# shubhamchandak94/HARC

Hardware: AMD Instinct MI355X
Metric: Mreads/s reorder+encode, 100 bp (higher is better)
Workload: dtype u64 (2-bit packed bases, XOR+popcount)

## Files before the change

harc_amd/csrc/stage2.hip:

```cpp
#include "devutil.h"
#include <time.h>
#include <algorithm>
#include <stdlib.h>

#define TUPLE_NONE 0xFFFFFFFFFFFFFFFFULL

struct S2Args {
    int L, W, W3, thresh_s, maxsearch;
    int ds[2], de[2], kbits[2];
    uint32_t M, S, T, q, nC;
    uint64_t total;
    const uint64_t *oreads;
    const uint8_t *flag, *pos, *rc;
    const uint32_t *order;
    const uint64_t *cand3;
    const uint32_t *cand_order;
    uint8_t *head;
    uint64_t *gstart;
    uint8_t *cons;
    const uint32_t *chead;
    const HashSlot *slots[2]; uint64_t cap[2]; const uint32_t *ids[2];
    unsigned long long *best;
    unsigned long long *bestbin[2];
    const uint32_t *bloom[2]; int bloom_shift[2];
    int bloom_lbits, bloom_nwin;
    const uint64_t *cons2;
    const uint64_t *cand2, *candN;
    uint4 *events;
    unsigned int *nevents; uint32_t maxevents;
    int trace;
    uint64_t col0, col1; uint32_t tile_base;
    const uint64_t *evwin;
    unsigned long long *cbb[2]; uint32_t *cpos[2], *ccnt[2]; unsigned long long *tminbin[2]; int compact;
    int binmax_on;
    unsigned long long *binmax[2];
};

__device__ __forceinline__ int base2_at(const uint64_t *r, int j) { return (int)((r[j >> 5] >> (2 * (j & 31))) & 3); }
__device__ __forceinline__ int pc_to_idx(int pc) { return ((pc & 1) << 1) | (pc >> 1); }
__device__ __forceinline__ int c3_at(const uint64_t *r, int W3, int j)
{
    const int off = 3 * j, wi = off >> 6, sh = off & 63;
    uint64_t v = r[wi] >> sh;
    if (sh > 61 && wi + 1 < W3) v |= r[wi + 1] << (64 - sh);
    return (int)(v & 7);
}
__device__ __forceinline__ int c3_to_idx5(int c3) { return c3 == 0 ? 0 : c3 == 4 ? 1 : c3 == 2 ? 2 : c3 == 6 ? 3 : 4; }
__device__ __forceinline__ int idx_to_c3(int idx) { return idx == 0 ? 0 : idx == 1 ? 4 : idx == 2 ? 2 : 6; }
__device__ __forceinline__ int comp5(int b) { return b == 4 ? 4 : 3 - b; }
__device__ __forceinline__ char enc_noise(int ref, int rd)
{
    const unsigned tabA = 0x32100, tabC = 0x32100, tabG = 0x30021, tabT = 0x30012;
    const unsigned t = ref == 0 ? tabA : ref == 1 ? tabC : ref == 2 ? tabG : tabT;
    return (char)('0' + ((t >> (4 * rd)) & 0xF));
}
__device__ __forceinline__ long long ub_le(const uint64_t *a, long long n, uint64_t x)
{
    long long lo = -1, hi = n;
    while (hi - lo > 1) { const long long mid = (lo + hi) >> 1; if (a[mid] <= x) lo = mid; else hi = mid; }
    return lo;
}

__global__ void k_cand3_from2(const uint64_t *reads2, const uint32_t *gather, uint32_t n, int L, int W, int W3, uint64_t *out)
{
    const size_t gid = harc_gid();
    if (gid >= (size_t)n * W3) return;
    const uint32_t i = (uint32_t)(gid / W3); const int w = (int)(gid % W3);
    const uint64_t *r = reads2 + (size_t)(gather ? gather[i] : i) * W;
    uint64_t v = 0;
    const int b0 = (64 * w) / 3, b1 = (64 * w + 63) / 3;
    for (int b = b0; b <= b1 && b < L; b++) {
        const uint64_t c3 = (uint64_t)(2 * base2_at(r, b));
        const int sh = 3 * b - 64 * w;
        v |= sh >= 0 ? (c3 << sh) : (c3 >> (-sh));
    }
    out[gid] = v;
}
__global__ void k_cand_order(const uint32_t *order_s, uint32_t S, uint32_t T, uint32_t *out)
{
    const uint32_t i = harc_gid32();
    if (i >= T) return;
    out[i] = i < S ? order_s[i] : i - S;
}
__global__ void k_key3(const uint64_t *cand3, uint32_t T, int W3, int off, int nbits, uint64_t *keys, uint32_t *ids)
{
    const uint32_t i = harc_gid32();
    if (i >= T) return;
    const uint64_t *r = cand3 + (size_t)i * W3;
    const int wi = off >> 6, sh = off & 63;
    uint64_t v = r[wi] >> sh;
    if (sh && wi + 1 < W3) v |= r[wi + 1] << (64 - sh);
    if (nbits < 64) v &= ((uint64_t)1 << nbits) - 1;
    keys[i] = v; ids[i] = i;
}
__global__ void k_count_big_bins(const HashSlot *slots, uint64_t cap, uint32_t maxsearch, unsigned long long *out)
{
    const uint64_t i = harc_gid();
    if (i >= cap) return;
    if ((slots[i].count & SLOT_CNT_MASK) > maxsearch) atomicAdd(out, 1ULL);
}

__global__ void k_heads1(const uint8_t *flag, uint32_t M, uint32_t q, uint8_t *head, uint32_t *hidx)
{
    const uint32_t i = harc_gid32();
    if (i >= M) return;
    const uint8_t h = (flag[i] == '0' || (i % q) == 0) ? 1 : 0;
    head[i] = h; hidx[i] = h ? i : 0;
}
__global__ void k_heads2(uint32_t M, uint8_t *head, const uint32_t *hmax, uint32_t *hidx)
{
    const uint32_t i = harc_gid32();
    if (i >= M) return;
// ... 249 lines not shown
    lh ^= lh >> 15; lh *= 0x85EBCA77u; lh ^= lh >> 13;
    *word = ((lh >> (32 - lbits)) << 4) | ((kh >> 6) & 15u);
    *sh0 = 4 * (int)(kh & 7u); *sh1 = 4 * (int)((kh >> 3) & 7u);
}
__global__ void k_bloom4_set(const uint64_t *keys, uint32_t n, uint32_t *bloom, int lbits, int nwin, int l, int nb)
{
    const uint32_t i = harc_gid32();
    if (i >= n) return;
    const uint64_t k = keys[i];
    uint64_t f = 0, r = 0;
    for (int b = 0; b < nb; b++) {
        const uint32_t c3 = (uint32_t)(k >> (3 * b)) & 7u;
        if (c3 & 1u) return;
        const uint64_t idx = ((c3 >> 2) & 1u) | (c3 & 2u);
        f |= idx << (2 * b); r |= (3u - idx) << (2 * (nb - 1 - b));
    }
    uint32_t w; int a, b;
    bloom4_pos(f, bloom4_minimizer(f, nwin), nwin, lbits, &w, &a, &b);
    atomicOr(&bloom[w], ((1u << l) << a) | ((1u << l) << b));
    bloom4_pos(r, bloom4_minimizer(r, nwin), nwin, lbits, &w, &a, &b);
    atomicOr(&bloom[w], ((4u << l) << a) | ((4u << l) << b));
}
__global__ void k_bloom4_items(const uint64_t *keys, uint32_t n, int lbits, int nwin, int l, int nb, uint32_t skip_tile, uint64_t *items)
{
    const uint32_t i = harc_gid32();
    if (i >= n) return;
    const uint64_t k = keys[i];
    uint64_t f = 0, r = 0; bool hasn = false;
    for (int b = 0; b < nb; b++) {
        const uint32_t c3 = (uint32_t)(k >> (3 * b)) & 7u;
        hasn |= (c3 & 1u) != 0;
        const uint64_t idx = ((c3 >> 2) & 1u) | (c3 & 2u);
        f |= idx << (2 * b); r |= (3u - idx) << (2 * (nb - 1 - b));
    }
    if (hasn) { items[2 * (size_t)i] = items[2 * (size_t)i + 1] = (uint64_t)skip_tile; return; }
    uint32_t w; int a, b;
    bloom4_pos(f, bloom4_minimizer(f, nwin), nwin, lbits, &w, &a, &b);
    items[2 * (size_t)i] = harc_bitmap_item(w, a + l, b + l);
    bloom4_pos(r, bloom4_minimizer(r, nwin), nwin, lbits, &w, &a, &b);
    items[2 * (size_t)i + 1] = harc_bitmap_item(w, a + 2 + l, b + 2 + l);
}
__global__ void k_words_differ(const uint32_t *a, const uint32_t *b, uint64_t nwords, unsigned long long *ndiff)
{
    const uint64_t i = harc_gid();
    const unsigned long long m = __ballot(i < nwords && a[i] != b[i]);
    if ((threadIdx.x & 63) == 0 && m) atomicAdd(ndiff, (unsigned long long)__popcll(m));
}
__global__ void k_cand2_from3(const uint64_t *cand3, uint32_t T, int L, int W, int W3, uint64_t *cand2, uint64_t *candN)
{
    const uint64_t gid = harc_gid();
    if (gid >= (uint64_t)T * W) return;
    const uint32_t i = (uint32_t)(gid / W); const int w = (int)(gid % W);
    const uint64_t *r = cand3 + (size_t)i * W3;
    (void)L;
    const int wi = (3 * w) >> 1;
    const uint64_t x0 = r[wi], x1 = wi + 1 < W3 ? r[wi + 1] : 0;
    uint64_t lo, hi;
    if (w & 1) { lo = (x0 >> 32) | (x1 << 32); hi = x1 >> 32; } else { lo = x0; hi = x1 & 0xFFFFFFFFull; }
    uint64_t a = 0, n = 0;
#pragma unroll
    for (int k = 0; k < 32; k++) {
        const uint64_t c3 = (k <= 20 ? (lo >> (3 * k)) : k == 21 ? ((lo >> 63) | (hi << 1)) : (hi >> (3 * k - 64))) & 7;
        a |= (c3 >> 1) << (2 * k);
        n |= ((c3 & 1) * 3) << (2 * k);
    }
    cand2[gid] = a; candN[gid] = n;
}
template <int W> __device__ __forceinline__ void cons_words(const uint64_t *cons2, uint64_t g, uint64_t (&cw)[W])
{
    const uint64_t bit = 2 * g, wi = bit >> 6; const int sh = (int)(bit & 63);
    uint64_t lo = cons2[wi];
#pragma unroll
    for (int w = 0; w < W; w++) { const uint64_t hi = cons2[wi + w + 1]; cw[w] = sh ? ((lo >> sh) | (hi << (64 - sh))) : lo; lo = hi; }
}

#define RSTRIP 8
#define RTILE (256 * RSTRIP)
static_assert(RTILE == CTILE, "the proposal kernels are launched on the consensus kernel's tiles");
template <int W> __device__ __forceinline__ void realign_probe(const S2Args &s, uint64_t x, int dir, int l, uint64_t key)
{
    uint32_t st = 0, cnt = 0;
    if (!dict_lookup_b(s.slots[l], s.cap[l], key, &st, &cnt)) return;
    const int L = s.L;
    const unsigned long long tp = (x << 2) | ((uint64_t)dir << 1) | (uint64_t)l;
    if (cnt & SLOT_BIG) {
        const unsigned int at = atomicAdd(s.nevents, 1u);
        if (at < s.maxevents) s.events[at] = make_uint4((uint32_t)tp, (uint32_t)(tp >> 32), st, cnt & SLOT_CNT_MASK);
        return;
    }
    uint64_t wv[W];
    {
        uint64_t cw[W];
        cons_words<W>(s.cons2, x, cw);
#pragma unroll
        for (int w = 0; w < W; w++) cw[w] &= lowmask_word(2 * L, w);
        if (dir) rc_words<W>(cw, L, wv);
        else {
#pragma unroll
            for (int w = 0; w < W; w++) wv[w] = cw[w];
        }
    }
    const bool emb = (cnt & SLOT_EMB) != 0;
    cnt &= SLOT_CNT_MASK;
    for (uint32_t t = 0; t < cnt; t++) {
        const uint32_t rid = emb ? st : s.ids[l][st + cnt - 1 - t];
        const uint64_t *a2 = s.cand2 + (size_t)rid * W, *n2 = s.candN + (size_t)rid * W;
        int hd = 0;
#pragma unroll
        for (int w = 0; w < W; w++) {
            const uint64_t av = a2[w], nv = n2[w];
            hd += __popcll((av ^ wv[w]) & ~nv) + __popcll(nv & 0x5555555555555555ULL) + __popcll(wv[w] & nv);
        }
        if (hd <= s.thresh_s) atomicMin(&s.best[rid], tp);
    }
}
#define RQCAP 4096
template <int W> __device__ __forceinline__ void realign_hit1(const S2Args &s, const uint8_t *tile, uint64_t X0, int tc, int p, int n)
{
    const int dir = p >> 1, l = p & 1;
    const uint64_t cpos = X0 + tc;
    const uint64_t off = dir ? (uint64_t)(s.L - 1 - s.de[l]) : (uint64_t)s.ds[l];
    if (cpos < off) return;
    const uint64_t x = cpos - off;
    if (x < s.col0 || x >= s.col1 || !(s.cons[x] & 4)) return;
    uint64_t key = 0;
    if (dir) for (int b = 0; b < n; b++) key |= (uint64_t)idx_to_c3(3 - (tile[tc + n - 1 - b] & 3)) << (3 * b);
    else for (int b = 0; b < n; b++) key |= (uint64_t)idx_to_c3(tile[tc + b] & 3) << (3 * b);
    realign_probe<W>(s, x, dir, l, key);
}
template <int W, int NWIN> __global__ __launch_bounds__(256) void k_realign_propose1(S2Args s)
{
    __shared__ uint32_t tile32[(RTILE + 64 + 8) / 4];
    __shared__ uint16_t queue[RQCAP];
    __shared__ uint2 lookup[RTILE];
    __shared__ unsigned int qn;
    uint8_t *tile = reinterpret_cast<uint8_t *>(tile32);
    const uint64_t X0 = (uint64_t)(blockIdx.x + s.tile_base) * RTILE;
    const int n = s.de[0] - s.ds[0] + 1;
    const int ntile = RTILE + n + NWIN + 1;
    for (int d = threadIdx.x; d < (ntile + 3) / 4; d += 256) {
        const uint64_t g = X0 + 4ull * d;
        uint32_t v = 0;
        if (g + 4 <= s.total) v = *reinterpret_cast<const uint32_t *>(s.cons + g);
        else for (int k = 0; k < 4; k++) if (g + k < s.total) v |= (uint32_t)s.cons[g + k] << (8 * k);
        tile32[d] = v;
    }
    if (threadIdx.x == 0) qn = 0;
    __syncthreads();
    const int t0 = threadIdx.x * RSTRIP;
    uint64_t k = 0;
    for (int b = 0; b < n; b++) k |= (uint64_t)(tile[t0 + b] & 3) << (2 * b);
    const uint32_t *bloom = s.bloom[0]; const int lbits = s.bloom_lbits;
    constexpr int NK = RSTRIP + (NWIN > 0 ? NWIN - 1 : 0);
    uint64_t keys[RSTRIP]; uint32_t mm[NK];
#pragma unroll
    for (int c = 0; c < NK; c++) {
        if (c < RSTRIP) keys[c] = k;
        mm[c] = bloom4_mmer(k);
        k = (k >> 2) | ((uint64_t)(tile[t0 + c + n] & 3) << (2 * (n - 1)));
    }
#pragma unroll
    for (int c = 0; c < RSTRIP; c++) {
        uint32_t mz = 0xFFFFFFFFu;
#pragma unroll
        for (int i = 0; i < NWIN; i++) mz = mm[c + i] < mz ? mm[c + i] : mz;
        uint32_t w; int a, b;
        bloom4_pos(keys[c], mz, NWIN, lbits, &w, &a, &b);
        lookup[t0 + c] = make_uint2(w, (uint32_t)a | ((uint32_t)b << 8));
    }
    __syncthreads();
#pragma unroll
    for (int c = 0; c < RSTRIP; c++) {
        const int col = c * 256 + (int)threadIdx.x;
        if (X0 + col < s.total) {
            const uint2 lk = lookup[col];
            const uint32_t v = bloom[lk.x];
            uint32_t m = (v >> (lk.y & 0xFFu)) & (v >> (lk.y >> 8)) & 15u;
            while (m) {
                const int p = __builtin_ctz(m); m &= m - 1;
                const unsigned int at = atomicAdd(&qn, 1u);
                if (at < RQCAP) queue[at] = (uint16_t)(col | (p << 12));
                else realign_hit1<W>(s, tile, X0, col, p, n);
            }
        }
    }
    __syncthreads();
    const unsigned int nq = qn < RQCAP ? qn : RQCAP;
    for (unsigned int i = threadIdx.x; i < nq; i += 256) { const uint16_t e = queue[i]; realign_hit1<W>(s, tile, X0, e & 0xFFF, e >> 12, n); }
}

template <int W> __global__ __launch_bounds__(256) void k_realign_propose(S2Args s)
{
    __shared__ uint32_t tile32[(RTILE + 256 + 8) / 4];
    uint8_t *tile = reinterpret_cast<uint8_t *>(tile32);
    const uint64_t X0 = (uint64_t)(blockIdx.x + s.tile_base) * RTILE;
    const int L = s.L;
    const int ntile = RTILE + L + 1;
    for (int d = threadIdx.x; d < (ntile + 3) / 4; d += 256) {
        const uint64_t g = X0 + 4ull * d;
        uint32_t v = 0;
        if (g + 4 <= s.total) v = *reinterpret_cast<const uint32_t *>(s.cons + g);
        else for (int k = 0; k < 4; k++) if (g + k < s.total) v |= (uint32_t)s.cons[g + k] << (8 * k);
        tile32[d] = v;
    }
    __syncthreads();
    const int t0 = threadIdx.x * RSTRIP;
    if (X0 + t0 >= s.total) return;
    const int n0 = s.de[0] - s.ds[0] + 1, n1 = s.de[1] - s.ds[1] + 1;
    const uint64_t m0 = (n0 * 3 < 64) ? ((1ULL << (3 * n0)) - 1) : ~0ULL, m1 = (n1 * 3 < 64) ? ((1ULL << (3 * n1)) - 1) : ~0ULL;
    uint64_t kf0 = 0, kf1 = 0, kr0 = 0, kr1 = 0;
    for (int b = 0; b < n0; b++) {
        kf0 |= (uint64_t)idx_to_c3(tile[t0 + s.ds[0] + b] & 3) << (3 * b);
        kr0 |= (uint64_t)idx_to_c3(3 - (tile[t0 + L - 1 - s.ds[0] - b] & 3)) << (3 * b);
    }
    for (int b = 0; b < n1; b++) {
        kf1 |= (uint64_t)idx_to_c3(tile[t0 + s.ds[1] + b] & 3) << (3 * b);
        kr1 |= (uint64_t)idx_to_c3(3 - (tile[t0 + L - 1 - s.ds[1] - b] & 3)) << (3 * b);
    }
    for (int c = 0; c < RSTRIP; c++) {
        const int tx = t0 + c;
        const uint64_t x = X0 + tx;
        if (x >= s.total) break;
        if (x >= s.col0 && x < s.col1 && (tile[tx] & 4)) {
            const uint64_t keys[4] = { kf0, kf1, kr0, kr1 };
            bool pass[4];
#pragma unroll
            for (int k = 0; k < 4; k++) {
                const int l = k & 1;
                const uint64_t b = mix64(keys[k] ^ 0x9E3779B97F4A7C15ULL) >> s.bloom_shift[l];
                pass[k] = (s.bloom[l][b >> 5] >> (b & 31)) & 1u;
            }
#pragma unroll
            for (int k = 0; k < 4; k++) if (pass[k]) realign_probe<W>(s, x, k >> 1, k & 1, keys[k]);
        }
        kf0 = (kf0 >> 3) | ((uint64_t)idx_to_c3(tile[tx + 1 + s.de[0]] & 3) << (3 * (n0 - 1)));
        kf1 = (kf1 >> 3) | ((uint64_t)idx_to_c3(tile[tx + 1 + s.de[1]] & 3) << (3 * (n1 - 1)));
        kr0 = ((kr0 << 3) & m0) | (uint64_t)idx_to_c3(3 - (tile[tx + L - s.ds[0]] & 3));
        kr1 = ((kr1 << 3) & m1) | (uint64_t)idx_to_c3(3 - (tile[tx + L - s.ds[1]] & 3));
    }
}

#define EV_DONE 0xFFFFFFFEu
__global__ void k_ev_key_tuple(const uint4 *ev, uint32_t nev, uint64_t *key, uint32_t *idx)
{
    const uint32_t i = harc_gid32();
    if (i >= nev) return;
    const uint4 e = ev[i];
    key[i] = (uint64_t)e.x | ((uint64_t)e.y << 32); idx[i] = i;
}
__global__ void k_ev_key_bin(const uint4 *ev, const uint32_t *idx, uint32_t nev, uint64_t *key)
{
    const uint32_t i = harc_gid32();
    if (i >= nev) return;
    const uint4 e = ev[idx[i]];
    key[i] = ((uint64_t)(e.x & 1u) << 32) | e.z;
}
__global__ void k_ev_gather(const uint4 *ev, const uint32_t *perm, uint32_t nev, uint4 *out)
{
    const uint32_t i = harc_gid32();
    if (i < nev) out[i] = ev[perm[i]];
}
__global__ __launch_bounds__(256) void k_ev_windows(S2Args s, const uint4 *ev, uint32_t nev, uint64_t *win, uint32_t kbase)
{
    __shared__ uint8_t sc3[4][256];
    const int wv = threadIdx.x >> 6, lane = threadIdx.x & 63;
    const uint32_t e = kbase + blockIdx.x * 4 + wv;
    if (e >= nev) return;
    const uint4 v = ev[e];
    const unsigned long long tp = (unsigned long long)v.x | ((unsigned long long)v.y << 32);
    const uint64_t x = tp >> 2; const int dir = (int)((tp >> 1) & 1), L = s.L;
    for (int b = lane; b < L; b += 64) {
// ... 769 lines not shown
    auto lap = [&](const char *what) { if (trace2) { (void)hipStreamSynchronize(c->stream); struct timespec t; clock_gettime(CLOCK_MONOTONIC, &t); fprintf(stderr, "[stage II%s] %s: %.1f ms\n", part ? " (partitioned)" : "", what, (t.tv_sec - tl0.tv_sec) * 1e3 + (t.tv_nsec - tl0.tv_nsec) * 1e-6); tl0 = t; } };

    S2Args a; memset(&a, 0, sizeof a);
    a.L = L; a.W = W; a.W3 = W3; a.thresh_s = P.thresh_s; a.maxsearch = P.maxsearch;
    if (L > 50) { a.ds[0] = 0; a.de[0] = 20; a.ds[1] = 21; a.de[1] = 41; }
    else { a.ds[0] = 0; a.de[0] = 20 * L / 50; a.ds[1] = 20 * L / 50 + 1; a.de[1] = 41 * L / 50; }
    for (int l = 0; l < 2; l++) a.kbits[l] = 3 * (a.de[l] - a.ds[l] + 1);
    a.M = M; a.S = S; a.T = T;
    a.q = 1u + (uint32_t)((M - 1u) / E);
    if (a.q == 0) a.q = 1;
    a.oreads = c->d_oreads; a.flag = c->d_flag; a.pos = c->d_pos; a.rc = c->d_rc; a.order = c->d_order;
    const uint32_t i0 = (uint32_t)((uint64_t)e0 * a.q > M ? M : (uint64_t)e0 * a.q), i1 = e1 >= E ? M : (uint32_t)((uint64_t)e1 * a.q > M ? M : (uint64_t)e1 * a.q);

    uint32_t *order_out = nullptr, *orderN_out = nullptr;
    RC_TRY(dalloc(c, &order_out, (size_t)(i1 - i0) + (size_t)S + 1)); RC_TRY(dalloc(c, &orderN_out, (size_t)NN + 1));
    c->d_s2_order = c->d_s2_orderN = nullptr; c->n_s2_order = c->n_s2_orderN = 0;
    PoolScope s2_scope(c);
    const bool want_digest = P.stream_digest != 0;
    unsigned long long *d_digest = nullptr;
    c->have_digest = false;
    if (want_digest) { RC_TRY(dalloc(c, &d_digest, 4)); HIP_TRY(hipMemsetAsync(d_digest, 0, 32, c->stream)); }

    uint64_t *cand3 = nullptr; uint32_t *cand_order = nullptr; unsigned long long *best = nullptr;
    RC_TRY(dalloc(c, &cand3, (size_t)T * W3 + 1)); RC_TRY(dalloc(c, &cand_order, (size_t)T + 1)); RC_TRY(dalloc(c, &best, (size_t)T + 1));
    if (S) {
        if (c->d_sreads) hipLaunchKernelGGL(k_cand3_from2, G256((size_t)S * W3), c->d_sreads, (const uint32_t *)nullptr, S, L, W, W3, cand3);
        else hipLaunchKernelGGL(k_cand3_from2, G256((size_t)S * W3), c->d_reads, c->d_order_s, S, L, W, W3, cand3);
    }
    if (NN) HIP_TRY(hipMemcpyAsync(cand3 + (size_t)S * W3, c->d_nreads3, (size_t)NN * W3 * 8, hipMemcpyDeviceToDevice, c->stream));
    if (T) hipLaunchKernelGGL(k_cand_order, G256(T), c->d_order_s, S, T, cand_order);
    HIP_TRY(hipMemsetAsync(best, 0xFF, ((size_t)T + 1) * 8, c->stream));
    a.cand3 = cand3; a.cand_order = cand_order; a.best = best;
    uint8_t *head = nullptr; uint32_t *u1 = nullptr; uint64_t *gstart = nullptr; uint32_t *chead = nullptr;
    RC_TRY(dalloc(c, &head, (size_t)M + 1)); RC_TRY(dalloc(c, &u1, (size_t)M + 1)); RC_TRY(dalloc(c, &gstart, (size_t)M + 1));
    uint32_t nC = 0; uint64_t total = 0;
    if (M) {
        PoolScope cscope(c);
        uint32_t *u0 = nullptr; uint64_t *d64 = nullptr;
        RC_TRY(dalloc(c, &u0, (size_t)M + 1)); RC_TRY(dalloc(c, &d64, (size_t)M + 1));
        hipLaunchKernelGGL(k_heads1, G256(M), c->d_flag, M, a.q, head, u0);
        RC_TRY(prim_incl_max_u32(c, u0, u1, M));
        hipLaunchKernelGGL(k_heads2, G256(M), M, head, u1, u0);
        RC_TRY(prim_excl_scan_u32(c, u0, u1, M));
        hipLaunchKernelGGL(k_col_steps, G256(M), head, c->d_pos, M, L, d64);
        RC_TRY(prim_incl_scan_u64(c, d64, gstart, M));
        uint32_t lastcid = 0, lasthead = 0; uint64_t lastg = 0;
        HIP_TRY(hipMemcpyAsync(&lastcid, u1 + (M - 1), 4, hipMemcpyDeviceToHost, c->stream));
        HIP_TRY(hipMemcpyAsync(&lasthead, u0 + (M - 1), 4, hipMemcpyDeviceToHost, c->stream));
        HIP_TRY(hipMemcpyAsync(&lastg, gstart + (M - 1), 8, hipMemcpyDeviceToHost, c->stream));
        HIP_TRY(hipStreamSynchronize(c->stream));
        nC = lastcid + lasthead; total = lastg + (uint64_t)L;
    }
    RC_TRY(dalloc(c, &chead, (size_t)nC + 1));
    if (M) hipLaunchKernelGGL(k_contig_heads, G256(M), head, u1, M, chead);
    a.head = head; a.gstart = gstart; a.chead = chead; a.nC = nC; a.total = total;
    c->C.contigs = nC; c->C.seq_bases = total;
    std::vector<uint64_t> sh_col(E + 1, total), seq_off(E, 0), seq_nb(E, 0), seq_tl(E, 0);
    for (uint32_t e = 0; e <= E; e++) {
        const uint64_t st = (uint64_t)e * a.q; const uint32_t i = e == E ? M : (uint32_t)(st > M ? M : st);
        if (i >= M) { sh_col[e] = total; continue; }
        HIP_TRY(hipMemcpyAsync(&sh_col[e], gstart + i, 8, hipMemcpyDeviceToHost, c->stream));
    }
    HIP_TRY(hipStreamSynchronize(c->stream));
    const uint64_t col0 = sh_col[e0], col1 = sh_col[e1];
    a.col0 = col0; a.col1 = col1; a.tile_base = (uint32_t)(col0 / CTILE);
    if (part) c->C.seq_bases = col1 - col0;
    lap("contig structure (all reads, on every rank)");
    uint64_t *cons2 = nullptr;
    const uint64_t ncw = (total + 31) / 32;
    RC_TRY(dalloc(c, &cons2, (size_t)ncw + 2 * W + 4));
    HIP_TRY(hipMemsetAsync(cons2 + ncw, 0, ((size_t)2 * W + 4) * 8, c->stream));
    a.cons2 = cons2;
    uint64_t seq_total = 0;
    for (uint32_t e = e0; e < e1; e++) { const uint64_t cc = sh_col[e + 1] - sh_col[e]; seq_nb[e] = cc / 4; seq_tl[e] = cc % 4; seq_off[e] = seq_total; seq_total += (seq_nb[e] + seq_tl[e] + 15) & ~15ull; }
    uint8_t *seqpk = nullptr; RC_TRY(dalloc(c, &seqpk, (size_t)seq_total + 64));
    PoolScope ascope(c);
    uint64_t *cand2 = nullptr, *candN = nullptr;
    RC_TRY(dalloc(c, &cand2, (size_t)T * W + 1)); RC_TRY(dalloc(c, &candN, (size_t)T * W + 1));
    if (T) hipLaunchKernelGGL(k_cand2_from3, G256((size_t)T * W), (const uint64_t *)cand3, T, L, W, W3, cand2, candN);
    a.cand2 = cand2; a.candN = candN;
    a.maxevents = 1u << 20;
    if (c->s2_events_hint > a.maxevents) a.maxevents = c->s2_events_hint;
    if (const char *e = getenv("HARC_AMD_MAXEVENTS")) { a.maxevents = (uint32_t)strtoul(e, nullptr, 10); if (a.maxevents < 1) a.maxevents = 1; }
    RC_TRY(dalloc(c, &a.events, (size_t)a.maxevents)); RC_TRY(dalloc(c, &a.nevents, 4));
    HIP_TRY(hipMemsetAsync(a.nevents, 0, 16, c->stream));

    lap("  candidates: 3-bit store, 2-bit copies");
    DictDev dict[2];
    unsigned long long *d_big = nullptr; RC_TRY(dalloc(c, &d_big, 1));
    HIP_TRY(hipMemsetAsync(d_big, 0, 8, c->stream));
    uint32_t *bloom[2] = { nullptr, nullptr }; int bloom_shift[2] = { 63, 63 };
    const bool bloom4 = a.kbits[0] == a.kbits[1] && !getenv("HARC_AMD_BLOOM1");
    bool bloom4_tiled = false;
    int bloom_per_key = 16;
    if (const char *e = getenv("HARC_AMD_BLOOMBITS")) { bloom_per_key = atoi(e); if (bloom_per_key < 1) bloom_per_key = 1; }
    if (T) {
        RC_TRY(harc_dict_alloc(c, &dict[0], T, 0)); RC_TRY(harc_dict_alloc(c, &dict[1], T, dict[0].cap));
        dict[0].bigthresh = dict[1].bigthresh = (uint32_t)P.maxsearch < 32u ? (uint32_t)P.maxsearch : 32u;
        int lb = 16; while (lb < 36 && (1ULL << lb) < (unsigned long long)bloom_per_key * T) lb++;
        if (bloom4) {
            RC_TRY(dalloc(c, &bloom[0], ((size_t)1 << (lb - 3)) + 1));
            bloom4_tiled = getenv("HARC_AMD_S2BLOOM_TILED") ? atoi(getenv("HARC_AMD_S2BLOOM_TILED")) != 0 : (((size_t)1 << (lb - 3)) * 4 >= ((size_t)64 << 20));
            if ((uint64_t)T * 4 > 0xFFFFFFFFull || harc_bitmap_tiles((uint64_t)1 << (lb - 3)) + 1 >= (1u << BL_PART_BITS)) bloom4_tiled = false;
            if (!bloom4_tiled) HIP_TRY(hipMemsetAsync(bloom[0], 0, ((size_t)1 << (lb - 3)) * 4, c->stream));
            bloom[1] = bloom[0]; bloom_shift[0] = bloom_shift[1] = 64 - lb;
            a.bloom_lbits = lb - 7;
            a.bloom_nwin = (a.kbits[0] / 3 == 21 && !getenv("HARC_AMD_BLOOM4_HASHED")) ? 21 - BLOOM4_M + 1 : 0;
        } else for (int l = 0; l < 2; l++) {
            RC_TRY(dalloc(c, &bloom[l], ((size_t)1 << (lb - 5)) + 1));
            HIP_TRY(hipMemsetAsync(bloom[l], 0, ((size_t)1 << (lb - 5)) * 4, c->stream));
            bloom_shift[l] = 64 - lb;
        }
        PoolScope kscope(c);
        uint64_t *k0 = nullptr; uint32_t *i0k = nullptr; uint64_t *items = nullptr, *items_tmp = nullptr;
        RC_TRY(dalloc(c, &k0, T)); RC_TRY(dalloc(c, &i0k, T));
        const uint64_t b4words = (uint64_t)1 << (lb - 3);
        if (bloom4 && bloom4_tiled) { RC_TRY(dalloc(c, &items, (size_t)T * 4 + 1)); RC_TRY(dalloc(c, &items_tmp, (size_t)T * 4 + 1)); }
        for (int l = 0; l < 2; l++) {
            hipLaunchKernelGGL(k_key3, G256(T), cand3, T, W3, 3 * a.ds[l], a.kbits[l], k0, i0k);
            if (bloom4 && bloom4_tiled) hipLaunchKernelGGL(k_bloom4_items, G256(T), (const uint64_t *)k0, T, a.bloom_lbits, a.bloom_nwin, l, a.kbits[l] / 3, harc_bitmap_tiles(b4words), items + (size_t)l * 2 * T);
            else if (bloom4) hipLaunchKernelGGL(k_bloom4_set, G256(T), (const uint64_t *)k0, T, bloom[0], a.bloom_lbits, a.bloom_nwin, l, a.kbits[l] / 3);
            else hipLaunchKernelGGL(k_bloom_set, G256(T), (const uint64_t *)k0, T, bloom[l], bloom_shift[l]);
            lap("  keys, bitmap items");
            RC_TRY(harc_dict_build(c, &dict[l], k0, i0k, T, (unsigned)a.kbits[l]));
            hipLaunchKernelGGL(k_count_big_bins, G256(dict[l].cap), dict[l].slots, dict[l].cap, (uint32_t)P.maxsearch, d_big);
            lap("  dictionary built");
        }
        if (bloom4 && bloom4_tiled) {
            RC_TRY(harc_bitmap_from_items(c, items, items_tmp, (size_t)T * 4, b4words, bloom[0]));
            lap("  combined bitmap from sorted items");
            if (getenv("HARC_AMD_S2BLOOM_VERIFY")) {
                uint32_t *ref = nullptr; unsigned long long *nd = nullptr, hnd = 0;
                RC_TRY(dalloc(c, &ref, (size_t)b4words + 1)); RC_TRY(dalloc(c, &nd, 1));
                HIP_TRY(hipMemsetAsync(ref, 0, (size_t)b4words * 4, c->stream)); HIP_TRY(hipMemsetAsync(nd, 0, 8, c->stream));
                for (int l = 0; l < 2; l++) {
                    hipLaunchKernelGGL(k_key3, G256(T), cand3, T, W3, 3 * a.ds[l], a.kbits[l], k0, i0k);
                    hipLaunchKernelGGL(k_bloom4_set, G256(T), (const uint64_t *)k0, T, ref, a.bloom_lbits, a.bloom_nwin, l, a.kbits[l] / 3);
                }
                hipLaunchKernelGGL(k_words_differ, harc_grid256(b4words), dim3(256), 0, c->stream, (const uint32_t *)ref, (const uint32_t *)bloom[0], b4words, nd);
                HIP_TRY(hipMemcpyAsync(&hnd, nd, 8, hipMemcpyDeviceToHost, c->stream));
                HIP_TRY(hipStreamSynchronize(c->stream));
                if (hnd) { harc_set_error("stage II bitmap built by tiles differs from the one built with atomics in %llu words", hnd); return HARC_AMD_EINTERNAL; }
            }
        }
        HIP_TRY(hipStreamSynchronize(c->stream));
    }
    for (int l = 0; l < 2; l++) { a.slots[l] = dict[l].slots; a.cap[l] = dict[l].cap; a.ids[l] = dict[l].ids; a.bloom[l] = bloom[l]; a.bloom_shift[l] = bloom_shift[l]; }
    lap("candidates and their dictionaries (all candidates, on every rank)");

    uint8_t *h_seq = nullptr;
    struct CopyJoin { hipStream_t s; ~CopyJoin() { (void)hipStreamSynchronize(s); } } copy_join{ c->copy_stream };
    uint8_t *cons = nullptr; RC_TRY(dalloc(c, &cons, (size_t)total + 8));
    a.cons = cons;
    unsigned int nev = 0;
    if (col1 > col0) {
        unsigned long long *cinfo = nullptr; RC_TRY(dalloc(c, &cinfo, (size_t)nC + 1));
        hipLaunchKernelGGL(k_contig_info, G256(nC), a, cinfo);
        const uint32_t ntiles = (uint32_t)((col1 + CTILE - 1) / CTILE) - a.tile_base;
        uint32_t *tlo = nullptr, *thi = nullptr; RC_TRY(dalloc(c, &tlo, (size_t)ntiles + 1)); RC_TRY(dalloc(c, &thi, (size_t)ntiles + 1));
        hipLaunchKernelGGL(k_consensus_tiles, G256(ntiles), a, ntiles, tlo, thi);
        uint32_t *tovf = nullptr; RC_TRY(dalloc(c, &tovf, (size_t)ntiles + 1));
        HIP_TRY(hipMemsetAsync(tovf, 0, (size_t)ntiles * 4, c->stream));
        hipLaunchKernelGGL(k_consensus<CSHALLOW>, dim3(ntiles), dim3(CTHREADS), (size_t)CCHUNK * (W * 8 + 4), c->stream, a, (const uint32_t *)u1, (const unsigned long long *)cinfo, T ? 1 : 0,
                           (const uint32_t *)tlo, (const uint32_t *)thi, tovf);
        hipLaunchKernelGGL(k_consensus<CPLANES>, dim3(ntiles), dim3(CTHREADS), (size_t)CCHUNK * (W * 8 + 4), c->stream, a, (const uint32_t *)u1, (const unsigned long long *)cinfo, T ? 1 : 0,
                           (const uint32_t *)tlo, (const uint32_t *)thi, tovf);
        { const uint64_t w0 = col0 / 32, w1 = (col1 + 31) / 32; hipLaunchKernelGGL(k_pack_cons2, G256(w1 - w0), (const uint8_t *)a.cons, total, w0, w1 - w0, cons2); }
        {
            const uint64_t soff = seq_total;
            for (uint32_t e = e0; e < e1; e++) {
                const uint64_t cc0 = sh_col[e];
                if (seq_nb[e]) hipLaunchKernelGGL(k_pack2_bytes, G256(seq_nb[e]), cons + cc0, seq_nb[e], seqpk + seq_off[e]);
                if (seq_tl[e]) hipLaunchKernelGGL(k_bases_to_ascii, G256(seq_tl[e]), cons + cc0 + 4 * seq_nb[e], seq_tl[e], seqpk + seq_off[e] + seq_nb[e]);
            }
            HIP_TRY(hipGetLastError());
            if (want_digest) for (uint32_t e = e0; e < e1; e++) RC_TRY(digest_range(c, seqpk + seq_off[e], seq_nb[e] + seq_tl[e], 0x100 + e, d_digest + 0));
            RC_TRY(harc_host_alloc(c, (void **)&h_seq, (size_t)soff));
            HIP_TRY(hipEventRecord(c->ev_copy, c->stream));
            HIP_TRY(hipStreamWaitEvent(c->copy_stream, c->ev_copy, 0));
            if (soff) HIP_TRY(hipMemcpyAsync(h_seq, seqpk, (size_t)soff, hipMemcpyDeviceToHost, c->copy_stream));
        }
        if (T) {
            const dim3 rg(ntiles);
            auto propose = [&]() {
                switch (W) {
#define REALIGN_CASE(WW) case WW: if (bloom4 && a.bloom_nwin) hipLaunchKernelGGL((k_realign_propose1<WW, 21 - BLOOM4_M + 1>), rg, dim3(256), 0, c->stream, a); \
                                 else if (bloom4) hipLaunchKernelGGL((k_realign_propose1<WW, 0>), rg, dim3(256), 0, c->stream, a); \
                                 else hipLaunchKernelGGL((k_realign_propose<WW>), rg, dim3(256), 0, c->stream, a); break;
                    REALIGN_CASE(1) REALIGN_CASE(2) REALIGN_CASE(3) REALIGN_CASE(4) REALIGN_CASE(5) REALIGN_CASE(6) REALIGN_CASE(7) REALIGN_CASE(8)
#undef REALIGN_CASE
                }
            };
            propose();
            HIP_TRY(hipMemcpyAsync(&nev, a.nevents, 4, hipMemcpyDeviceToHost, c->stream));
            HIP_TRY(hipStreamSynchronize(c->stream));
            { const uint64_t want = (uint64_t)nev + nev / 4; c->s2_events_hint = want > 0xFFFFFFFFull ? 0xFFFFFFFFu : (uint32_t)want; }
            if (nev > a.maxevents) {
                a.maxevents = nev;
                RC_TRY(dalloc(c, &a.events, (size_t)a.maxevents));
                HIP_TRY(hipMemsetAsync(a.nevents, 0, 16, c->stream));
                propose();
                HIP_TRY(hipMemcpyAsync(&nev, a.nevents, 4, hipMemcpyDeviceToHost, c->stream));
                HIP_TRY(hipStreamSynchronize(c->stream));
                if (nev > a.maxevents) { harc_set_error("stage II: event count changed between two identical passes (%u > %u)", nev, a.maxevents); return HARC_AMD_EINTERNAL; }
            }
        }
    }
    HIP_TRY(hipGetLastError());
    unsigned long long *d_bdig = nullptr;
    auto best_digest = [&](const char *what) -> int {
        if (!getenv("HARC_AMD_TRACE") || !T) return HARC_AMD_OK;
        if (!d_bdig) RC_TRY(dalloc(c, &d_bdig, 2));
        unsigned long long hv = 0;
        HIP_TRY(hipMemsetAsync(d_bdig, 0, 8, c->stream));
        RC_TRY(digest_range(c, best, (uint64_t)T * 8, 0xBE57ull, d_bdig));
        HIP_TRY(hipMemcpyAsync(&hv, d_bdig, 8, hipMemcpyDeviceToHost, c->stream));
        HIP_TRY(hipStreamSynchronize(c->stream));
        fprintf(stderr, "[stage II] digest of the claims %s: %016llx (%u probes into large bins)\n", what, hv, nev);
        return HARC_AMD_OK;
    };
    RC_TRY(best_digest("after the proposals"));
    lap("consensus + read_seq + proposals (this rank's columns)");
    uint64_t *evwin = nullptr;
    if (nev) {
        RC_TRY(dalloc(c, &evwin, (size_t)nev * W3 + 1));
        WAVE_PER_ITEM(nev, hipLaunchKernelGGL(k_ev_windows, dim3(nb_), dim3(256), 0, c->stream, a, (const uint4 *)a.events, nev, evwin, kb_));
    }
    if (cm && T) {
        RC_TRY(cm->allreduce_min_u64(c, best, (size_t)T));
        RC_TRY(cm->wait(c, "all-reduce of the singleton / N-read claims"));
        std::vector<uint64_t> allnev((size_t)cm->world);
        { const uint64_t mine = nev; RC_TRY(cm->allgather_u64(c, &mine, 1, allnev.data())); }
        uint64_t tot = 0; for (uint64_t x : allnev) tot += x;
        if (tot > 0xFFFFFFFFull) { harc_set_error("stage II: more than 2^32 probes into large bins"); return HARC_AMD_EINVAL; }
        if (tot) {
            uint4 *ev_all = nullptr; uint64_t *win_all = nullptr;
            RC_TRY(dalloc(c, &ev_all, (size_t)tot + 1)); RC_TRY(dalloc(c, &win_all, (size_t)tot * W3 + 1));
            std::vector<size_t> so[2], sb[2], ro[2], rb[2];
            for (int k = 0; k < 2; k++) { so[k].assign(cm->world, 0); sb[k].resize(cm->world); ro[k].resize(cm->world); rb[k].resize(cm->world); }
            uint64_t acc = 0;
            for (int p = 0; p < cm->world; p++) {
                sb[0][p] = (size_t)nev * 16; sb[1][p] = (size_t)nev * W3 * 8;
                ro[0][p] = (size_t)acc * 16; rb[0][p] = (size_t)allnev[p] * 16; ro[1][p] = (size_t)acc * W3 * 8; rb[1][p] = (size_t)allnev[p] * W3 * 8;
                acc += allnev[p];
            }
            const void *sp[2] = { a.events, evwin }; void *rp[2] = { ev_all, win_all };
            const size_t *sop[2] = { so[0].data(), so[1].data() }, *sbp[2] = { sb[0].data(), sb[1].data() }, *rop[2] = { ro[0].data(), ro[1].data() }, *rbp[2] = { rb[0].data(), rb[1].data() };
            RC_TRY(cm->alltoallv(c, 2, sp, sop, sbp, rp, rop, rbp));
            RC_TRY(cm->wait(c, "all-gather of the probes into large bins"));
            a.events = ev_all; evwin = win_all; nev = (unsigned int)tot;
        } else nev = 0;
    }
    a.evwin = evwin;
    lap("all-reduce of the claims, probes into large bins gathered");
    if (nev) {
        unsigned int *d_changed = nullptr; uint32_t *estart = nullptr, *lastver = nullptr; unsigned long long *binmin[2] = { nullptr, nullptr };
        if (total >> (EV_TBITS - 2)) { harc_set_error("stage II: more than 2^%d consensus columns", EV_TBITS - 2); return HARC_AMD_EINVAL; }
        RC_TRY(dalloc(c, &d_changed, 8)); RC_TRY(dalloc(c, &estart, (size_t)nev + 1)); RC_TRY(dalloc(c, &lastver, (size_t)nev + 1));
        HIP_TRY(hipMemsetAsync(estart, 0xFF, ((size_t)nev + 1) * 4, c->stream));
        HIP_TRY(hipMemsetAsync(lastver, 0xFF, ((size_t)nev + 1) * 4, c->stream));
        for (int l = 0; l < 2; l++) { RC_TRY(dalloc(c, &binmin[l], 2 * ((size_t)T + 1))); HIP_TRY(hipMemsetAsync(binmin[l], 0xFF, 2 * ((size_t)T + 1) * 8, c->stream)); }
        a.binmax_on = !(getenv("HARC_AMD_S2_RANGE") && atoi(getenv("HARC_AMD_S2_RANGE")) == 0);
        for (int l = 0; l < 2; l++) { RC_TRY(dalloc(c, &a.binmax[l], 2 * ((size_t)T + 1))); HIP_TRY(hipMemsetAsync(a.binmax[l], 0, 2 * ((size_t)T + 1) * 8, c->stream)); }
        const bool trace = getenv("HARC_AMD_TRACE") != nullptr, nochase = getenv("HARC_AMD_S2_NOCHASE") != nullptr;
        a.trace = trace ? 1 : 0;
        struct timespec tw0; clock_gettime(CLOCK_MONOTONIC, &tw0);
        uint32_t *perm = nullptr, *rank = nullptr, *seglen = nullptr, *order2 = nullptr, *firsts = nullptr, *looklist = nullptr; unsigned int maxrank = 0, *d_nlist = nullptr, nfirsts = 0;
        uint32_t rhi0 = 64, range_end[32];
        if (const char *e = getenv("HARC_AMD_S2_RANK0")) { const int v = atoi(e); rhi0 = v < 1 ? 1u : (uint32_t)v; }
        for (int k = 0; k < 32; k++) range_end[k] = nev;
// ... 314 lines not shown
```

Baseline: 695.7.

## Overlay realign queue on lookup LDS, batch bloom loads and queue pushes

The realign proposal kernel now places its hit queue in the same shared memory as the lookup table, which cuts per-block LDS use so more blocks can be resident. All eight bloom words per thread are loaded up front, and hits are packed into a bitmask and pushed with one atomicAdd per group instead of one per hit. When the queue fills, the kernel drains it and loops rather than running the probe inline. It also adds an assume on L to narrow register use in the probe, plus env knobs for queue cap and LDS padding. The drain loop adds extra block-wide syncs, and the batched loads raise register pressure.

```diff
diff --git a/harc_amd/csrc/stage2.hip b/harc_amd/csrc/stage2.hip
--- a/harc_amd/csrc/stage2.hip
+++ b/harc_amd/csrc/stage2.hip
@@ -28,6 +28,7 @@
     const uint64_t *cand2, *candN;
     uint4 *events;
     unsigned int *nevents; uint32_t maxevents;
+    uint32_t qcap;
     int trace;
     uint64_t col0, col1; uint32_t tile_base;
     const uint64_t *evwin;
@@ -443,6 +444,7 @@
     uint32_t st = 0, cnt = 0;
     if (!dict_lookup_b(s.slots[l], s.cap[l], key, &st, &cnt)) return;
     const int L = s.L;
+    __builtin_assume(L > 32 * (W - 1) && L <= 32 * W);
     const unsigned long long tp = (x << 2) | ((uint64_t)dir << 1) | (uint64_t)l;
     if (cnt & SLOT_BIG) {
         const unsigned int at = atomicAdd(s.nevents, 1u);
@@ -492,9 +494,10 @@
 template <int W, int NWIN> __global__ __launch_bounds__(256) void k_realign_propose1(S2Args s)
 {
     __shared__ uint32_t tile32[(RTILE + 64 + 8) / 4];
-    __shared__ uint16_t queue[RQCAP];
     __shared__ uint2 lookup[RTILE];
     __shared__ unsigned int qn;
+    static_assert(RQCAP * sizeof(uint16_t) <= sizeof(lookup), "the queue lies over the lookup table");
+    uint16_t *queue = reinterpret_cast<uint16_t *>(lookup);
     uint8_t *tile = reinterpret_cast<uint8_t *>(tile32);
     const uint64_t X0 = (uint64_t)(blockIdx.x + s.tile_base) * RTILE;
     const int n = s.de[0] - s.ds[0] + 1;
@@ -509,45 +512,66 @@
     if (threadIdx.x == 0) qn = 0;
     __syncthreads();
     const int t0 = threadIdx.x * RSTRIP;
-    uint64_t k = 0;
-    for (int b = 0; b < n; b++) k |= (uint64_t)(tile[t0 + b] & 3) << (2 * b);
     const uint32_t *bloom = s.bloom[0]; const int lbits = s.bloom_lbits;
-    constexpr int NK = RSTRIP + (NWIN > 0 ? NWIN - 1 : 0);
-    uint64_t keys[RSTRIP]; uint32_t mm[NK];
-#pragma unroll
-    for (int c = 0; c < NK; c++) {
-        if (c < RSTRIP) keys[c] = k;
-        mm[c] = bloom4_mmer(k);
-        k = (k >> 2) | ((uint64_t)(tile[t0 + c + n] & 3) << (2 * (n - 1)));
-    }
+    {
+        uint64_t k = 0;
+        for (int b = 0; b < n; b++) k |= (uint64_t)(tile[t0 + b] & 3) << (2 * b);
+        constexpr int NK = RSTRIP + (NWIN > 0 ? NWIN - 1 : 0);
+        uint64_t keys[RSTRIP]; uint32_t mm[NK];
+#pragma unroll
+        for (int c = 0; c < NK; c++) {
+            if (c < RSTRIP) keys[c] = k;
+            mm[c] = bloom4_mmer(k);
+            k = (k >> 2) | ((uint64_t)(tile[t0 + c + n] & 3) << (2 * (n - 1)));
+        }
+#pragma unroll
+        for (int c = 0; c < RSTRIP; c++) {
+            uint32_t mz = 0xFFFFFFFFu;
+#pragma unroll
+            for (int i = 0; i < NWIN; i++) mz = mm[c + i] < mz ? mm[c + i] : mz;
+            uint32_t w; int a, b;
+            bloom4_pos(keys[c], mz, NWIN, lbits, &w, &a, &b);
+            lookup[t0 + c] = make_uint2(w, (uint32_t)a | ((uint32_t)b << 8));
+        }
+    }
+    __syncthreads();
+    uint2 lk[RSTRIP];
+#pragma unroll
+    for (int c = 0; c < RSTRIP; c++) lk[c] = lookup[c * 256 + (int)threadIdx.x];
+    uint32_t v[RSTRIP];
+#pragma unroll
+    for (int c = 0; c < RSTRIP; c++) v[c] = bloom[lk[c].x];
+    const uint32_t ncol = s.total - X0 < RTILE ? (uint32_t)(s.total - X0) : (uint32_t)RTILE;
+    uint32_t m = 0;
 #pragma unroll
     for (int c = 0; c < RSTRIP; c++) {
-        uint32_t mz = 0xFFFFFFFFu;
-#pragma unroll
-        for (int i = 0; i < NWIN; i++) mz = mm[c + i] < mz ? mm[c + i] : mz;
-        uint32_t w; int a, b;
-        bloom4_pos(keys[c], mz, NWIN, lbits, &w, &a, &b);
-        lookup[t0 + c] = make_uint2(w, (uint32_t)a | ((uint32_t)b << 8));
+        const uint32_t h = (v[c] >> (lk[c].y & 0xFFu)) & (v[c] >> (lk[c].y >> 8)) & 15u;
+        m |= (c * 256 + threadIdx.x < ncol ? h : 0u) << (4 * c);
     }
     __syncthreads();
-#pragma unroll
-    for (int c = 0; c < RSTRIP; c++) {
-        const int col = c * 256 + (int)threadIdx.x;
-        if (X0 + col < s.total) {
-            const uint2 lk = lookup[col];
-            const uint32_t v = bloom[lk.x];
-            uint32_t m = (v >> (lk.y & 0xFFu)) & (v >> (lk.y >> 8)) & 15u;
-            while (m) {
-                const int p = __builtin_ctz(m); m &= m - 1;
-                const unsigned int at = atomicAdd(&qn, 1u);
-                if (at < RQCAP) queue[at] = (uint16_t)(col | (p << 12));
-                else realign_hit1<W>(s, tile, X0, col, p, n);
+    constexpr int NPUSH = W >= 5 ? RSTRIP : 1, PBITS = 4 * RSTRIP / NPUSH;
+    const unsigned int qcap = s.qcap;
+    for (;;) {
+#pragma unroll
+        for (int g = 0; g < NPUSH; g++) {
+            const uint32_t gmask = PBITS == 32 ? 0xFFFFFFFFu : ((1u << (PBITS & 31)) - 1u) << (PBITS * g & 31);
+            uint32_t h = m & gmask;
+            if (h) {
+                unsigned int at = atomicAdd(&qn, (unsigned int)__popc(h));
+                while (h && at < qcap) {
+                    const int b = __builtin_ctz(h); h &= h - 1;
+                    queue[at++] = (uint16_t)(((b >> 2) * 256 + (int)threadIdx.x) | ((b & 3) << 12));
+                }
+                m = (m & ~gmask) | h;
             }
         }
-    }
-    __syncthreads();
-    const unsigned int nq = qn < RQCAP ? qn : RQCAP;
-    for (unsigned int i = threadIdx.x; i < nq; i += 256) { const uint16_t e = queue[i]; realign_hit1<W>(s, tile, X0, e & 0xFFF, e >> 12, n); }
+        __syncthreads();
+        const unsigned int nq = qn < qcap ? qn : qcap;
+        for (unsigned int i = threadIdx.x; i < nq; i += 256) { const uint16_t e = queue[i]; realign_hit1<W>(s, tile, X0, e & 0xFFF, e >> 12, n); }
+        if (!__syncthreads_or(m != 0)) break;
+        if (threadIdx.x == 0) qn = 0;
+        __syncthreads();
+    }
 }
 
 template <int W> __global__ __launch_bounds__(256) void k_realign_propose(S2Args s)
@@ -1483,6 +1507,8 @@
     a.maxevents = 1u << 20;
     if (c->s2_events_hint > a.maxevents) a.maxevents = c->s2_events_hint;
     if (const char *e = getenv("HARC_AMD_MAXEVENTS")) { a.maxevents = (uint32_t)strtoul(e, nullptr, 10); if (a.maxevents < 1) a.maxevents = 1; }
+    a.qcap = RQCAP;
+    if (const char *e = getenv("HARC_AMD_S2_QCAP")) { const long q = strtol(e, nullptr, 10); a.qcap = q < 1 ? 1u : q > RQCAP ? (uint32_t)RQCAP : (uint32_t)q; }
     RC_TRY(dalloc(c, &a.events, (size_t)a.maxevents)); RC_TRY(dalloc(c, &a.nevents, 4));
     HIP_TRY(hipMemsetAsync(a.nevents, 0, 16, c->stream));
 
@@ -1583,10 +1609,11 @@
         }
         if (T) {
             const dim3 rg(ntiles);
+            const size_t rp1_pad = getenv("HARC_AMD_S2_LDSPAD") ? (size_t)strtoul(getenv("HARC_AMD_S2_LDSPAD"), nullptr, 10) : 0;
             auto propose = [&]() {
                 switch (W) {
-#define REALIGN_CASE(WW) case WW: if (bloom4 && a.bloom_nwin) hipLaunchKernelGGL((k_realign_propose1<WW, 21 - BLOOM4_M + 1>), rg, dim3(256), 0, c->stream, a); \
-                                 else if (bloom4) hipLaunchKernelGGL((k_realign_propose1<WW, 0>), rg, dim3(256), 0, c->stream, a); \
+#define REALIGN_CASE(WW) case WW: if (bloom4 && a.bloom_nwin) hipLaunchKernelGGL((k_realign_propose1<WW, 21 - BLOOM4_M + 1>), rg, dim3(256), rp1_pad, c->stream, a); \
+                                 else if (bloom4) hipLaunchKernelGGL((k_realign_propose1<WW, 0>), rg, dim3(256), rp1_pad, c->stream, a); \
                                  else hipLaunchKernelGGL((k_realign_propose<WW>), rg, dim3(256), 0, c->stream, a); break;
                     REALIGN_CASE(1) REALIGN_CASE(2) REALIGN_CASE(3) REALIGN_CASE(4) REALIGN_CASE(5) REALIGN_CASE(6) REALIGN_CASE(7) REALIGN_CASE(8)
 #undef REALIGN_CASE
```

Result: no change. 691.0 (-0.7%).
